# ziatdinovmax/GPim

Hardware: AMD Instinct MI355X
Metric: GP fit+predict grid-points/sec (higher is better)
Workload: dtype f64; 1 GPU; C2: 256x256 synthetic twisted-lattice image, 25% observed (N=16384, M=65536, d=2), Matern52 exact GP, T=100 Adam its (lr 0.1) + predict; one image per GPU; N=16384, M=65536, kernel=Matern52

## Files before the change

### gpim_amd/csrc/api.hip

```cpp
#include <math.h>
#include <stdio.h>
#include <string.h>
#include <stdlib.h>
#include <algorithm>
#include <chrono>
#include <atomic>
#include <mutex>
#include "common.hpp"
#include "border.hpp"
#include "vgp.hpp"
#include "sm.hpp"
#include "sample.hpp"
#include "acq.hpp"

static thread_local std::string g_err;
void gpim_set_error(const std::string& s) { g_err = s; }

int deal_chunk(int ntiles) { return std::max(1, std::min(64, ntiles / 512)); }
#define EAGER_MIN_PANELS 12


static inline int64_t mat_doubles(const gpimhip_ctx* h, int64_t elements) { return h->fp32 ? (elements + 1) / 2 : elements; }

static void ws_release_matrix(gpimhip_ctx* h) {
// ... 525 lines not shown
            if (graph) (void)hipGraphDestroy(graph);
            graph = nullptr;
            exec = nullptr;
            (void)hipGetLastError();
        }
    }
    RunAhead ra(h, h->np, loop.run_ahead);
    if (!exec) {
        for (int t = 0; t < T && !ra.stop(t); ++t) GP_TRY(iteration());
        return finish_and_check(h);
    }
    hipError_t le = hipSuccess;
    for (int t = 0; t < T && le == hipSuccess && !ra.stop(t); ++t) le = hipGraphLaunch(exec, h->stream);
    const int rc = finish_and_check(h);
    (void)hipGraphExecDestroy(exec);
    (void)hipGraphDestroy(graph);
    HIP_TRY(le);
    return rc;
}

extern "C" {

const char* gpimhip_last_error(void) { return g_err.c_str(); }

int gpimhip_shutdown(void) {
    std::lock_guard<std::mutex> lock(g_side_mutex);
    for (auto& S : g_side) {
        if (S.capture) (void)hipStreamDestroy(S.capture);
        S = SideStreams();
    }
    g_side_generation.fetch_add(1);
    return GPIMHIP_OK;
}
int gpimhip_version(void) { return 100; }

int gpimhip_create(gpimhip_handle* out, int device, void* hip_stream) {
    if (!out) return GPIMHIP_E_BADARG;
    HIP_TRY(hipSetDevice(device));
    gpimhip_ctx* h = new gpimhip_ctx();
    h->device = device;
    h->stream = (hipStream_t)hip_stream;
    int rc = GPIMHIP_OK;
    if ((rc = h->theta1.alloc(h, 1)) || (rc = h->info.alloc(h, 4))) {
        delete h;
        return rc;
    }
    (void)hipMemsetAsync(h->info, 0, 4 * sizeof(int32_t), h->stream);
    *out = h;
    return GPIMHIP_OK;
}

int gpimhip_set_precision(gpimhip_handle h, int32_t bits) {
    if (!h || (bits != 32 && bits != 64)) return GPIMHIP_E_BADARG;
    const int want = bits == 32 ? 1 : 0;
    if (want == h->fp32) return GPIMHIP_OK;
    if (want && h->refl.mask) {
        gpim_set_error("the symmetry-reduced model computes in double precision: leave reflection mode (gpimhip_set_reflection(h, 0, ...)) first");
        return GPIMHIP_E_BADARG;
    }
    HIP_TRY(hipSetDevice(h->device));
    HIP_TRY(hipStreamSynchronize(h->stream));
    ws_release_matrix(h);
    ws_release_predict(h);
    sample_release(h);
    ivr_release(h);
    h->fp32 = want;
    return GPIMHIP_OK;
}

int gpimhip_destroy(gpimhip_handle h) {
    if (!h) return GPIMHIP_OK;
    (void)hipSetDevice(h->device);
    (void)hipStreamSynchronize(h->stream);
    vfe_release(h);
    kron_release(h);
    vgp_release(h);
    pkron_release(h);
    sm_release(h);
    border_release(h);
    sample_release(h);
    ivr_release(h);
    ws_release_matrix(h);
    ws_release_predict(h);
    dev_release(h, h->keys, h->sel_scratch, h->acq_tmp, h->refine, h->bc, h->theta1, h->info, h->loo_tiles);
    if (h->plan.d_tiles) (void)hipFree(h->plan.d_tiles);
    step_plan_release(h);
    dist_plan_release(h);
    for (auto e : h->ra_ev)
        if (e) (void)hipEventDestroy(e);
    if (h->pinned_info) (void)hipHostFree(h->pinned_info);
    delete h;
    return GPIMHIP_OK;
}

int64_t gpimhip_workspace_bytes(gpimhip_handle h) {
    if (!h) return 0;
    const BorderWs* w = bws(h);
    return h->bytes + (w && w->sub ? w->sub->bytes : 0) + sample_bytes(h);
}

int gpimhip_timing_enable(gpimhip_handle h, int enable) {
    if (!h) return GPIMHIP_E_BADARG;
    h->timing = enable != 0;
    return GPIMHIP_OK;
}

int gpimhip_timing_read(gpimhip_handle h, int stage, double* total_ms, int64_t* count) {
    if (!h || stage < 0 || stage > 6 || !total_ms || !count) return GPIMHIP_E_BADARG;
    HIP_TRY(hipStreamSynchronize(h->stream));
    double tot = 0.0;
    for (auto& pr : h->ev[stage]) {
        float ms = 0.f;
        (void)hipEventElapsedTime(&ms, pr.first, pr.second);
        tot += ms;
        (void)hipEventDestroy(pr.first);
        (void)hipEventDestroy(pr.second);
    }
    *total_ms = tot;
    *count = (int64_t)h->ev[stage].size();
    h->ev[stage].clear();
    return GPIMHIP_OK;
}

int gpimhip_fit_completed(gpimhip_handle h) { return h ? h->fit_completed : 0; }

int gpimhip_sync(gpimhip_handle h) {
    if (!h) return GPIMHIP_E_BADARG;
    HIP_TRY(hipStreamSynchronize(h->stream));
    return GPIMHIP_OK;
}

int gpimhip_kmat(gpimhip_handle h, const gpimhip_model_t* m, const double* X, int64_t N, const double* Z,
                 int64_t M, const double* theta, double diag_add, double* out, int64_t ld) {
    FP64_ONLY(h);
    if (!h || !X || !theta || !out || N < 1) return GPIMHIP_E_BADARG;
    GP_TRY(check_model(m));
    HIP_TRY(hipSetDevice(h->device));
    const bool sym = (Z == nullptr);
    const int64_t Mv = sym ? N : M;
    if (Mv < 1 || ld < Mv) return GPIMHIP_E_BADARG;
    h->nbatch = 1;
    GP_TRY(launch_theta_raw(h, m, theta));
    const int64_t rp = pad_to(N, NB), cp = pad_to(Mv, NB);
    GP_TRY(ws_ensure_predict(h, rp, cp));
    const int64_t kld = h->ks_cols + 16;
    GP_TRY(launch_kmat(h, m, X, N, sym ? nullptr : Z, Mv, h->theta1, diag_add, 0, h->Ks, kld, rp, cp, sym ? 1 : 0, 0, 0,
                       0, 0));
    HIP_TRY(hipMemcpy2DAsync(out, (size_t)ld * sizeof(double), h->Ks, (size_t)kld * sizeof(double),
                             (size_t)Mv * sizeof(double), (size_t)N, hipMemcpyDeviceToDevice, h->stream));
    return GPIMHIP_OK;
}

int gpimhip_potrf(gpimhip_handle h, double* A, int64_t n, int64_t ld, int32_t* info) {
    FP64_ONLY(h);
    if (!h || !A || n < 1 || ld < n || !info) return GPIMHIP_E_BADARG;
    HIP_TRY(hipSetDevice(h->device));
    h->nbatch = 1;
    GP_TRY(ws_ensure(h, n));
    const int64_t np = h->np;
    HIP_TRY(hipMemsetAsync(info, 0, sizeof(int32_t), h->stream));
    GP_TRY(launch_pad_matrix_in(h, A, n, ld, h->A, np));
    GP_TRY(launch_potrf(h, h->A, np, np, info));
    GP_TRY(launch_pad_matrix_out_lower(h, h->A, np, A, n, ld));
    return GPIMHIP_OK;
}

static int fit_impl(gpimhip_ctx* h, const gpimhip_model_t* m, const double* X, int64_t x_bs, const double* y,
                    int64_t N, int B, double* u, double lr, int32_t T, double* hist_out, double* loss_out,
                    Objective obj = OBJ_NLL) {
    read_finalize_knob(h);
    HIP_TRY(hipSetDevice(h->device));
    h->nbatch = B;
    HIP_TRY(hipMemsetAsync(h->info, 0, sizeof(int32_t), h->stream));
    HIP_TRY(hipMemsetAsync(h->info + 1, 0x7f, sizeof(int32_t), h->stream));
    h->fit_completed = T;
    if (T == 0) return GPIMHIP_OK;
    GP_TRY(upload_bc_table(h, lr, T));
    if (use_small_path(N) && !h->refl.mask && obj == OBJ_NLL) {
        GP_TRY(launch_fit_small(h, m, X, x_bs, y, (int)N, u, h->bc, h->bc + T, T, hist_out, loss_out, nullptr));
        return finish_and_check(h);
    }
    GP_TRY(ws_ensure_padded(h, N));
    if (obj == OBJ_LOO) GP_TRY(loo_obj_ensure(h));
    if (border_on(h)) GP_TRY(border_ensure(h));
    HIP_TRY(hipMemsetAsync(h->adam_m, 0, (size_t)B * MAXP * sizeof(double), h->stream));
    HIP_TRY(hipMemsetAsync(h->adam_v, 0, (size_t)B * MAXP * sizeof(double), h->stream));
    HIP_TRY(hipMemsetAsync(h->iter, 0, (size_t)B * sizeof(int32_t), h->stream));
    HIP_TRY(hipMemsetAsync(h->fin_counter, 0, (size_t)B * sizeof(uint32_t), h->stream));
    GP_TRY(launch_pad_copy(h, y, N, h->ypad, h->np));
    const bool carry = !h->refl.mask && !h->no_fused_finalize;
    if (carry) GP_TRY(launch_theta(h, m, u));
    const IterTable tab{{h->iter, h->bc, T, hist_out, loss_out}, carry};
    const AdamStep st = adam_step_init();
    return run_fit_iterations(h, T, FIT_LOOP_DENSE,
                              [&] { return loss_grad_at_u(h, m, X, x_bs, N, u, 1, st, nullptr, nullptr, nullptr, &tab, obj); });
}


extern "C++" int64_t predict_chunk_cols(int64_t np, int B, int64_t M) {
    int64_t mc = std::min(pad_to(M, NB), std::max<int64_t>(NB, ((int64_t)1 << 27) / np / B / NB * NB));
    if (const char* e = getenv("GPIMHIP_PREDICT_CHUNK")) mc = std::min(mc, std::max<int64_t>(NB, atoll(e) / NB * NB));
    return mc;
}

extern "C++" int predict_cols(gpimhip_ctx* h, const PredictFamily& f, int64_t N, int B) {
    const int64_t np = h->np, M = f.M;
    const int nb = (int)(np / NB);
    if (f.fused && !h->fp32 && fused_predict_fits(np)) return f.fused();
    const int64_t mc = predict_chunk_cols(np, B, M);
    GP_TRY(ws_ensure_predict(h, np, mc));
    const bool bd = border_on(h);
    if (bd) GP_TRY(border_ensure_r(h, h->ks_cols));
    for (int64_t m0 = 0; m0 < M; m0 += mc) {
        const int64_t cnt = std::min(mc, M - m0), mcap = h->ks_cols;
        PredictChunk c{f.Xs + m0 * f.dim, m0, cnt, pad_to(cnt, NB), mcap, mcap + 16, cnt, nullptr};
        GP_TRY(f.slab(c));
        GP_TRY(launch_gemv_t(h, h->Ks, c.kld, np, c.cpad, h->alpha, h->mean_tmp, 0, np * c.kld, np, c.mcap));
        if (f.mean) GP_TRY(f.mean(c));
        if (f.var_on_domain && h->refl.var_count > 0 && !bd) c.nvar = std::max<int64_t>(0, std::min(cnt, h->refl.var_count - m0));
        if (c.nvar > 0) {
            GemmArgs g = gemm_args(h->A, h->ld, h->Ks, c.kld, nullptr, 0, 1.0, 0.0, h->pred_tiles, 0, h->np);
            if (c.nvar < c.cnt) g.cj_max = (int)((c.nvar + NB - 1) / NB);
            g.sB = np * c.kld;
            g.colpart = h->colpart;
            g.ld_colpart = c.mcap;
            g.sColpart = (int64_t)nb * c.mcap;
            g.ntiles = (int)h->pred_ntiles;
            g.chunk = deal_chunk(g.ntiles);
            g.rag = h->fp32 ? 0 : rag_of(N, np);
            { StageTimer t(h, 3); GP_TRY(launch_gemm(h, false, true, EPI_COLSUMSQ, g)); }
            if (bd) {
                BorderWs* w = bws(h);
                w->sub->stream = h->stream;
                const int64_t brows = (int64_t)(B / w->T) * np;
                GemmArgs gr = gemm_args(w->Y, w->mp, h->Ks, c.kld, w->R, w->r_cols, 1.0, 0.0, nullptr, 0, 0);
                gr.sA = brows * w->mp;
                gr.sB = brows * c.kld;
                gr.sC = w->mp * w->r_cols;
                gr.rect_rows = (int)(w->mp / NB);
                gr.rect_cols = (int)(c.cpad / NB);
                gr.ntiles = gr.rect_rows * gr.rect_cols;
                gr.kfix0 = 0;
                gr.kfix1 = (int)(brows / NB);
                gr.chunk = deal_chunk(gr.ntiles);
                GP_TRY(launch_gemm(w->sub, true, true, EPI_STORE, gr));
                GP_TRY(launch_border_colsumsq(h, w, c.cnt));
                c.radd = w->rsq;
            }
        }
        GP_TRY(f.finish(c));
    }
    return GPIMHIP_OK;
}

extern "C++" PredictFamily stationary_family(gpimhip_ctx* h, const gpimhip_model_t* m, const double* X, int64_t x_bs, int64_t N,
                                             int B, const double* Xs, int64_t M, double* mean_out, double* var_out) {
    PredictFamily f{m->dim, Xs, M};
    if (h->refl.mask) {
        const double scale = 1.0 / sqrt((double)(h->refl.nblocks_total > 0 ? h->refl.nblocks_total : B));
        f.var_on_domain = true;
        f.slab = [=](const PredictChunk& c) {
            return launch_kmat_refl(h, m, X, N, c.Z, c.cnt, h->theta, h->Ks, c.kld, h->np, c.cpad, 0, x_bs, 0, h->np * c.kld, scale);
        };
        f.finish = [=](const PredictChunk& c) {
            return launch_predict_coupled(h, c.mcap, (int)(h->np / NB), c.m0, c.cnt, c.nvar, c.mcap, mean_out, var_out, c.radd);
        };
        return f;
    }
    f.fused = [=] { return launch_predict_fused(h, m, X, x_bs, N, Xs, M, mean_out, var_out); };
    f.slab = [=](const PredictChunk& c) {
        return launch_kmat(h, m, X, N, c.Z, c.cnt, h->theta, 0.0, 0, h->Ks, c.kld, h->np, c.cpad, 0, 0, x_bs, 0, h->np * c.kld);
    };
    f.mean = [=](const PredictChunk& c) { return launch_copy_slice(h, h->mean_tmp, mean_out + c.m0, c.cnt, c.mcap, M); };
    f.finish = [=](const PredictChunk& c) { return launch_predict_var(h, c.mcap, (int)(h->np / NB), c.m0, c.cnt, var_out, M); };
    return f;
}

extern "C++" int model_state_at_u(gpimhip_ctx* h, const gpimhip_model_t* m, const double* X, int64_t x_bs, const double* y,
                                  int64_t N, int B, const double* u) {
    HIP_TRY(hipSetDevice(h->device));
    h->nbatch = B;
    GP_TRY(ws_ensure_padded(h, N));
    const int64_t np = h->np;
    HIP_TRY(hipMemsetAsync(h->info, 0, sizeof(int32_t), h->stream));
    GP_TRY(launch_pad_copy(h, y, N, h->ypad, np));
    if (border_on(h)) GP_TRY(border_ensure(h));
    GP_TRY(factor_at_u(h, m, X, x_bs, N, u));
    if (border_on(h)) {
        GP_TRY(launch_lauum(h, h->A, h->B, np, h->ld, rag_of(N, np)));
        GP_TRY(border_iter(h, N, false));
    }
    return GPIMHIP_OK;
}

static int predict_impl(gpimhip_ctx* h, const gpimhip_model_t* m, const double* X, int64_t x_bs, const double* y,
                        int64_t N, int B, const double* u, const double* Xs, int64_t M, double* mean_out,
                        double* var_out) {
    GP_TRY(model_state_at_u(h, m, X, x_bs, y, N, B, u));
    GP_TRY(predict_cols(h, stationary_family(h, m, X, x_bs, N, B, Xs, M, mean_out, var_out), N, B));
    return finish_and_check(h);
}

static int loss_grad_impl(gpimhip_ctx* h, const gpimhip_model_t* m, const double* X, const double* y, int64_t N, const double* u,
                          double* loss_out, double* grad_out, Objective obj) {
    read_finalize_knob(h);
    HIP_TRY(hipSetDevice(h->device));
    h->nbatch = 1;
    HIP_TRY(hipMemsetAsync(h->info, 0, sizeof(int32_t), h->stream));
    if (use_small_path(N) && obj == OBJ_NLL) {
        GP_TRY(launch_fit_small(h, m, X, 0, y, (int)N, const_cast<double*>(u), nullptr, nullptr, 0, nullptr,
                                loss_out, grad_out));
        return finish_and_check(h);
    }
    GP_TRY(ws_ensure_padded(h, N));
    if (obj == OBJ_LOO) GP_TRY(loo_obj_ensure(h));
    GP_TRY(launch_pad_copy(h, y, N, h->ypad, h->np));
    AdamStep st;
    memset(&st, 0, sizeof(st));
    GP_TRY(loss_grad_at_u(h, m, X, 0, N, const_cast<double*>(u), 0, st, loss_out, grad_out, nullptr, nullptr, obj));
    return finish_and_check(h);
}

int gpimhip_nll_grad(gpimhip_handle h, const gpimhip_model_t* m, const double* X, const double* y, int64_t N,
                     const double* u, double* loss_out, double* grad_out) {
    if (!h || !X || !y || !u || N < 1) return GPIMHIP_E_BADARG;
    GP_TRY(check_model(m));
    return loss_grad_impl(h, m, X, y, N, u, loss_out, grad_out, OBJ_NLL);
}

static int loo_objective_refused(const gpimhip_ctx* h, const char* who) {
    const char* why = h->fp32 ? "a single-precision handle (d = diag(S^-1) and the loss's log d cancel in float matrices: gpimhip_set_precision(h, 64))"
                    : border_on(h) ? "a border (the missing points couple the blocks: diag(S^-1) is no sum of the blocks' diagonals)"
                    : (h->refl.pb_off != 0 || h->refl.pb_stride != 1 || h->refl.raw || h->refl.nblocks_total) && h->refl.mask
                        ? "a shard of reflection blocks (the objective is not a sum over the blocks)"
                    : h->refl.mask ? "reflection mode (a lock-step batch of blocks: the held-out terms mix the blocks' diagonals)"
                                   : nullptr;
    if (!why) return GPIMHIP_OK;
    gpim_set_error(std::string(who) + ": the leave-one-out objective is the dense double-precision model's, one problem per call; refused on " + why);
    return GPIMHIP_E_BADARG;
}

int gpimhip_loo_grad(gpimhip_handle h, const gpimhip_model_t* m, const double* X, const double* y, int64_t N, const double* u,
                     double* loss_out, double* grad_out) {
    if (!h || !X || !y || !u || N < 1) return GPIMHIP_E_BADARG;
    GP_TRY(check_model(m));
    GP_TRY(loo_objective_refused(h, "gpimhip_loo_grad"));
    return loss_grad_impl(h, m, X, y, N, u, loss_out, grad_out, OBJ_LOO);
}

int gpimhip_fit_exact_loo(gpimhip_handle h, const gpimhip_model_t* m, const double* X, const double* y, int64_t N,
                          double* u_inout, double lr, int32_t T, double* hist_out, double* loss_out) {
    if (!h || !X || !y || !u_inout || N < 1 || T < 0) return GPIMHIP_E_BADARG;
    GP_TRY(check_model(m));
    GP_TRY(loo_objective_refused(h, "gpimhip_fit_exact_loo"));
    return fit_impl(h, m, X, 0, y, N, 1, u_inout, lr, T, hist_out, loss_out, OBJ_LOO);
}

int gpimhip_fit_exact(gpimhip_handle h, const gpimhip_model_t* m, const double* X, const double* y, int64_t N,
                      double* u_inout, double lr, int32_t T, double* hist_out, double* loss_out) {
    if (!h || !X || !y || !u_inout || N < 1 || T < 0) return GPIMHIP_E_BADARG;
    GP_TRY(check_model(m));
    return fit_impl(h, m, X, 0, y, N, 1, u_inout, lr, T, hist_out, loss_out);
}

int gpimhip_predict_exact(gpimhip_handle h, const gpimhip_model_t* m, const double* X, const double* y, int64_t N,
                          const double* u, const double* Xs, int64_t M, double* mean_out, double* var_out) {
    if (!h || !X || !y || !u || !Xs || M < 1 || N < 1 || !mean_out || !var_out) return GPIMHIP_E_BADARG;
    GP_TRY(check_model(m));
    return predict_impl(h, m, X, 0, y, N, 1, u, Xs, M, mean_out, var_out);
}

int gpimhip_fit_exact_batched(gpimhip_handle h, const gpimhip_model_t* m, const double* X, int64_t x_stride,
                              const double* y, int64_t N, int32_t B, double* u_inout, double lr, int32_t T,
                              double* hist_out, double* loss_out) {
    if (!h || !X || !y || !u_inout || N < 1 || T < 0 || B < 1 || B > 65535 ||
        (x_stride != 0 && x_stride < N * (m ? m->dim : 1)))
        return GPIMHIP_E_BADARG;
    GP_TRY(check_model(m));
    return fit_impl(h, m, X, x_stride, y, N, B, u_inout, lr, T, hist_out, loss_out);
}

int gpimhip_predict_exact_batched(gpimhip_handle h, const gpimhip_model_t* m, const double* X, int64_t x_stride,
// ... 137 lines not shown
```

### gpim_amd/csrc/common.hpp

```cpp
#pragma once
#include <hip/hip_runtime.h>
#include <stdint.h>
#include <functional>
#include <string>
#include <type_traits>
#include <vector>
#include <utility>
#include "../../include/gpimhip.h"

#define NB 128
#define GEMM_BK 16
#define MAXP GPIMHIP_MAX_PARAMS

void gpim_set_error(const std::string& s);

#define HIP_TRY(expr)                                                              \
    do {                                                                           \
        hipError_t _e = (expr);                                                    \
        if (_e != hipSuccess) {                                                    \
            gpim_set_error(std::string(#expr) + ": " + hipGetErrorString(_e));     \
            return GPIMHIP_E_HIP;                                                  \
        }                                                                          \
    } while (0)

// ... 97 lines not shown
    int64_t n_tiles = 0;
    std::vector<PlanRange> colfill;
    std::vector<PlanRange> upd_panel;
    std::vector<PlanRange> kinv_panel;
    PlanRange grad_tiles{0, 0};
    int rect_cols = 0;
    TileDesc* d_rect = nullptr;
    int64_t n_rect = 0;
};

struct ReflArgs {
    int mask;
    double twoc[GPIMHIP_MAX_DIM];
    const double* wts;
    int64_t n_total;
    int64_t var_count;
    int pb_off, pb_stride, nblocks_total, raw;
};
struct gpimhip_ctx {
    ReflArgs refl = {0, {0, 0, 0, 0}, nullptr, 0, 0, 0, 1, 0, 0};
    int device = 0;
    hipStream_t stream = nullptr;
    hipStream_t capture_stream = nullptr;
    bool capture_stream_tried = false;
    int side_generation = 0;
    int64_t np = 0;
    int64_t ld = 0;
    int nbatch = 1;
    int ws_batch = 0;
    DevBuf<double> A;
    DevBuf<double> B;
    DevBuf<double> Tm;
    DevBuf<double> dinv;
    DevBuf<double> dinvB;
    DevBuf<double> pcopy;
    DevBuf<double> ypad;
    DevBuf<double> z;
    DevBuf<double> alpha;
    DevBuf<double> logdet_part;
    DevBuf<double> grad_part;
    DevBuf<double> gemv_part;
    DevBuf<uint32_t> fin_counter;
    DevBuf<ThetaDev> theta;
    DevBuf<ThetaDev> theta1;
    DevBuf<int32_t> iter;
    DevBuf<double> adam_m;
    DevBuf<double> adam_v;
    DevBuf<int32_t> info;
    int64_t ks_rows = 0, ks_cols = 0, ks_batch = 0;
    struct PredList { int nc; DevBuf<TileDesc> tiles; };
    std::vector<PredList> pred_lists;
    DevBuf<double> Ks;
    DevBuf<double> colpart;
    DevBuf<double> mean_tmp;
    TileDesc* pred_tiles = nullptr;
    int64_t pred_ntiles = 0;
    int64_t bytes = 0;
    LinalgPlan plan;
    StepPlan splan, splan_inv;
    StepPlan splan_pair;
    DistPlan dplan;
    bool timing = false;
    std::vector<std::pair<hipEvent_t, hipEvent_t>> ev[7];
    DevBuf<double> bc;
    std::vector<double> bc_host;
    DevBuf<unsigned long long> keys;
    DevBuf<double> acq_tmp;
    DevBuf<char> sel_scratch;
    int fit_completed = 0;
    int32_t* pinned_info = nullptr;
    hipEvent_t ra_ev[2] = {nullptr, nullptr};
    void* vfe = nullptr;
    void* kron = nullptr;
    void* vgp = nullptr;
    void* pkron = nullptr;
    void* sm = nullptr;
    void* border = nullptr;
    void* sample = nullptr;
    void* ivr = nullptr;
    DevBuf<double> refine;
    DevBuf<double> loo_vec;
    DevBuf<TileDesc> loo_tiles;
    int loo_tiles_nb = 0;
    int fp32 = 0;
    bool no_fused_finalize = false;
};

template <typename T> int DevBuf<T>::alloc(gpimhip_ctx* h, int64_t count, const char* what) {
    void* q = nullptr;
    hipError_t e = hipMalloc(&q, (size_t)count * sizeof(T));
    if (e != hipSuccess) {
        if (what) (void)hipGetLastError();
        gpim_set_error(what ? std::string(what) : std::string("hipMalloc failed: ") + hipGetErrorString(e));
        return GPIMHIP_E_NOMEM;
    }
    p = (T*)q;
    cap = count;
    h->bytes += cap * (int64_t)sizeof(T);
    return GPIMHIP_OK;
}
template <typename T> void DevBuf<T>::release(gpimhip_ctx* h) {
    if (p) {
        (void)hipFree(p);
        h->bytes -= cap * (int64_t)sizeof(T);
    }
    p = nullptr;
    cap = 0;
}
template <typename T> int DevBuf<T>::grow(gpimhip_ctx* h, int64_t want) {
    if (cap >= want) return GPIMHIP_OK;
    HIP_TRY(hipStreamSynchronize(h->stream));
    release(h);
    return alloc(h, want);
}
template <typename... Bufs> static inline void dev_release(gpimhip_ctx* h, Bufs&... bufs) { (bufs.release(h), ...); }

struct BatchScope {
    gpimhip_ctx* h; int prev;
    BatchScope(gpimhip_ctx* h_, int nbatch) : h(h_), prev(h_->nbatch) { h->nbatch = nbatch; }
    ~BatchScope() { h->nbatch = prev; }
};

#define FP64_ONLY(h)                                                                                      \
    do {                                                                                                  \
        if ((h) && (h)->fp32) {                                                                           \
            gpim_set_error("this entry point needs a double-precision handle (gpimhip_set_precision(h, 64))"); \
            return GPIMHIP_E_BADARG;                                                                      \
        }                                                                                                 \
    } while (0)

static inline int64_t pad_to(int64_t n, int64_t m) { return (n + m - 1) / m * m; }
struct Carve {
    double* base;
    int64_t used = 0;
    explicit Carve(double* b) : base(b) {}
    template <typename T = double> T* take(int64_t doubles) {
        const int64_t off = (used + 1) & ~(int64_t)1;
        used = off + doubles;
        return base ? (T*)(base + off) : nullptr;
    }
};
static inline int rag_of(int64_t N, int64_t np) {
    const int64_t last = N - (np - NB);
    return (np >= 2 * NB && last > 0 && last <= 64) ? (int)(np / NB) : 0;
}

struct StageTimer {
    gpimhip_ctx* h; int stage; hipEvent_t e1 = nullptr;
    StageTimer(gpimhip_ctx* h_, int s) : h(h_), stage(s) {
        if (!h->timing) return;
        hipEvent_t e0;
        if (hipEventCreate(&e0) != hipSuccess || hipEventCreate(&e1) != hipSuccess) { e1 = nullptr; return; }
        (void)hipEventRecord(e0, h->stream);
        h->ev[stage].push_back({e0, e1});
    }
    ~StageTimer() { if (e1) (void)hipEventRecord(e1, h->stream); }
};

static inline int gemv_tri_rc(int64_t np) {
    const int64_t rc = ((np / 32 + NB - 1) / NB) * NB;
    return (int)(rc < NB ? NB : (rc > 1024 ? 1024 : rc));
}
static inline int gemv_tri_chunks(int64_t np) { return (int)((np + gemv_tri_rc(np) - 1) / gemv_tri_rc(np)); }
#define OUTER_W 4
int ws_ensure(gpimhip_ctx* h, int64_t N);
int ws_ensure_b(gpimhip_ctx* h, int64_t N, int B, int padded, bool matrices = true);
int ws_ensure_padded(gpimhip_ctx* h, int64_t N);
int ws_ensure_predict(gpimhip_ctx* h, int64_t np, int64_t mc);
int deal_chunk(int ntiles = 1 << 30);
void tri_tiles(std::vector<TileDesc>& tl, int nbr, int nc, bool lower);
void lower_patch_order(std::vector<TileDesc>& out, int lo, int hi, int kb0, int kb1);
int model_state_at_u(gpimhip_ctx* h, const gpimhip_model_t* m, const double* X, int64_t x_bs, const double* y, int64_t N,
                     int B, const double* u);
int solve_vectors(gpimhip_ctx* h, const gpimhip_model_t* m, const double* X, int64_t x_bs, int64_t N, bool defer_alpha = false);
int factor_at_u(gpimhip_ctx* h, const gpimhip_model_t* m, const double* X, int64_t x_bs, int64_t N, const double* u,
                bool theta_current = false, bool defer_alpha = false);
struct PredictChunk { const double* Z; int64_t m0, cnt, cpad, mcap, kld, nvar; const double* radd; };
struct PredictFamily {
    int dim; const double* Xs; int64_t M;
    bool var_on_domain = false;
    std::function<int()> fused;
    std::function<int(const PredictChunk&)> slab, mean, finish;
};
int64_t predict_chunk_cols(int64_t np, int B, int64_t M);
int predict_cols(gpimhip_ctx* h, const PredictFamily& f, int64_t N, int B);
PredictFamily stationary_family(gpimhip_ctx* h, const gpimhip_model_t* m, const double* X, int64_t x_bs, int64_t N, int B,
                                const double* Xs, int64_t M, double* mean_out, double* var_out);
void sample_release(gpimhip_ctx* h);
int64_t sample_bytes(const gpimhip_ctx* h);
void ivr_release(gpimhip_ctx* h);
int fit_prologue(gpimhip_ctx* h, double lr, int T, double* adam_m, double* adam_v, size_t adam_bytes, int32_t* iter);
int plan_ensure(gpimhip_ctx* h, int nb);
int check_model(const gpimhip_model_t* m);
int launch_potrf(gpimhip_ctx* h, double* A, int64_t np, int64_t ld, int32_t* info);
int launch_trtri(gpimhip_ctx* h, double* A, double* Tm, int64_t np, int64_t ld);
int launch_potrf_inv(gpimhip_ctx* h, double* A, double* Tm, int64_t np, int64_t ld, int32_t* info, int rag);
int launch_lauum(gpimhip_ctx* h, const double* A, double* B, int64_t np, int64_t ld, int rag);
int upload_bc_table(gpimhip_ctx* h, double lr, int T);
int finish_and_check(gpimhip_ctx* h);
struct FitLoop { bool dense_gates, run_ahead; };
static const FitLoop FIT_LOOP_DENSE = {true, true}, FIT_LOOP_PLAIN = {false, false};
int run_fit_iterations(gpimhip_ctx* h, int T, FitLoop loop, const std::function<int()>& iteration);
void vfe_release(gpimhip_ctx* h);
void kron_release(gpimhip_ctx* h);
void pkron_release(gpimhip_ctx* h);
int launch_potrf_steps(gpimhip_ctx* h, double* A, int64_t np, int64_t ld, int32_t* info, double* Tm = nullptr, int rag = 0);
int launch_potrf_steps_f32(gpimhip_ctx* h, double* A, int64_t np, int64_t ld, int32_t* info);
void step_plan_release(gpimhip_ctx* h);
int step_plan_ensure(gpimhip_ctx* h, int nb);
int step_plan_ensure_inv(gpimhip_ctx* h, int nb);
int step_plan_ensure_pair(gpimhip_ctx* h, int nb);
int launch_panel_chain(gpimhip_ctx* h, double* A, int64_t ld, int p0, int p1, int nb, const TileDesc* tiles,
                       const PlanRange* colfill, int32_t* info);
void dist_plan_release(gpimhip_ctx* h);
int launch_dist_pack(gpimhip_ctx* h, const double* P, int64_t ldp, int64_t r0, int64_t np, int w, const double* dinv,
                     int nblk, double* buf, int64_t ldb);
int launch_colsumsq_acc(gpimhip_ctx* h, const double* W, int64_t ldw, int rows, int64_t m, double* q);
int launch_dist_trsv(gpimhip_ctx* h, const double* P, int64_t ld, const double* D, int nblk, int backward, const double* r0,
                     const double* r1, double* out);
int launch_dist_rows_acc(gpimhip_ctx* h, const double* A, int64_t ld, int64_t rows, int w, const double* x, double* acc);
#define GEMV_T_MULTI_RC 1024
static inline int gemv_t_multi_chunks(int64_t nrows) { return (int)((nrows + GEMV_T_MULTI_RC - 1) / GEMV_T_MULTI_RC); }
int multi_group_width(int ncols);
int launch_dist_trsv_multi(gpimhip_ctx* h, const double* P, int64_t ld, const double* D, int nblk, int backward, const double* r0,
                           int64_t r0_cs, const double* r1, int64_t r1_cs, int64_t r1_chs, int nch, int ncols, double* out,
                           int64_t out_cs);
int launch_dist_rows_acc_multi(gpimhip_ctx* h, const double* A, int64_t ld, int64_t rows, int w, const double* x, int64_t x_cs,
                               int ncols, double* acc, int64_t acc_cs);
int launch_gemv_t_multi(gpimhip_ctx* h, const double* A, int64_t ld, int64_t nrows, int w, const double* x, int64_t x_cs,
                        int ncols, double* part);
int launch_theta_raw(gpimhip_ctx* h, const gpimhip_model_t* m, const double* raw);
int launch_kmat(gpimhip_ctx* h, const gpimhip_model_t* m, const double* X, int64_t N, const double* Z,
                int64_t M, const ThetaDev* theta, double diag_add, int use_theta_diag, double* out,
                int64_t ld, int64_t rows_pad, int64_t cols_pad, int sym, int lower_only, int64_t x_bs,
                int64_t z_bs, int64_t out_bs);
int launch_pad_copy(gpimhip_ctx* h, const double* src, int64_t n, double* dst, int64_t np);
int launch_diag_inv_copy(gpimhip_ctx* h, double* A, int64_t ld, int nb);
int launch_pad_matrix_in(gpimhip_ctx* h, const double* src, int64_t n, int64_t ld, double* dst, int64_t np);
int launch_pad_matrix_out_lower(gpimhip_ctx* h, const double* src, int64_t np, double* dst, int64_t n, int64_t ld);
int launch_trmv_lower(gpimhip_ctx* h, const double* L, int64_t ld, int64_t np, const double* y, double* z);
int launch_gemv_t(gpimhip_ctx* h, const double* A, int64_t ld, int64_t nrows, int64_t ncols, const double* x,
                  double* out, int tri, int64_t a_bs, int64_t x_bs, int64_t o_bs);
int launch_kres(gpimhip_ctx* h, const gpimhip_model_t* m, const double* X, int64_t x_bs, int64_t N, double* scratch,
                int S, double* res);
int launch_axpy(gpimhip_ctx* h, double* x, const double* d, int64_t n);
int launch_gemv_t_tri(gpimhip_ctx* h, const double* A, int64_t ld, int64_t np, const double* x, double* part, double* out);
int launch_kmat_refl(gpimhip_ctx* h, const gpimhip_model_t* m, const double* X, int64_t N, const double* Z, int64_t M,
                     const ThetaDev* theta, double* out, int64_t ld, int64_t rows_pad, int64_t cols_pad, int sym, int64_t x_bs,
                     int64_t z_bs, int64_t out_bs, double scale);
int launch_add_diag_theta(gpimhip_ctx* h, double* out, int64_t ld, int64_t row0, int64_t n, int64_t npad);
int launch_theta(gpimhip_ctx* h, const gpimhip_model_t* m, const double* u);
int launch_grad_reduce(gpimhip_ctx* h, const gpimhip_model_t* m, const double* Kinv, int64_t ld,
                       const double* X, int64_t N, int nb, const double* alpha, int64_t x_bs);
int launch_grad_reduce_fin(gpimhip_ctx* h, const gpimhip_model_t* m, const double* X, int64_t x_bs, int64_t N,
                           bool alpha_deferred, double* u, int do_adam, AdamStep st, const FinalizeOut& out, int carry_theta);
int launch_finalize(gpimhip_ctx* h, const gpimhip_model_t* m, int64_t N, int64_t np, double* u, int do_adam,
                    AdamStep st, const FinalizeOut& out, int carry_theta = 0);
int launch_finalize_vec(gpimhip_ctx* h, const gpimhip_model_t* m, int64_t N, int64_t np, double* u, int do_adam, AdamStep st,
                        const FinalizeOut& out, int carry_theta, const double* z, const double* zb);
int launch_grad_reduce_loo(gpimhip_ctx* h, const gpimhip_model_t* m, const double* Kinv, int64_t ld, const double* X, int64_t N,
                           int nb, const double* alpha, const double* rvec);
int loo_obj_ensure(gpimhip_ctx* h);
int loo_grad_at_u(gpimhip_ctx* h, const gpimhip_model_t* m, const double* X, int64_t N, double* u, int do_adam, AdamStep st,
                  const FinalizeOut& out, bool theta_carried);
int launch_grad_reduce_tiles(gpimhip_ctx* h, const gpimhip_model_t* m, const double* Kinv, int64_t ld, const double* X,
                             int64_t N, int64_t np, const double* alpha, const TileDesc* tiles, int ntile, double* part);
int launch_sum7(gpimhip_ctx* h, const double* part, int ntile, double* S);
int launch_grad_reduce_refl(gpimhip_ctx* h, const gpimhip_model_t* m, const double* Kinv, int64_t ld, const double* X,
                            int64_t N, int nb, const double* alpha, int64_t x_bs);
int launch_finalize_coupled(gpimhip_ctx* h, const gpimhip_model_t* m, int64_t N, int64_t np, double* u, int do_adam,
                            AdamStep st, const FinalizeOut& out, const double* border_scal = nullptr);
int launch_coupled_sums(gpimhip_ctx* h, int64_t np, double* out11);
int launch_dist_finalize_dev(gpimhip_ctx* h, const gpimhip_model_t* m, int64_t N, const double* red, const double* quad,
                             double* u, int do_adam, AdamStep st, double* loss_out, double* grad_out, double* hist_row);
int launch_dist_finalize(gpimhip_ctx* h, const gpimhip_model_t* m, int64_t N, const double* S, double q2, double lg,
                         double* u, int do_adam, AdamStep st, double* loss_out, double* grad_out, double* hist_row);
int launch_predict_var(gpimhip_ctx* h, int64_t ldp, int nb, int64_t m0, int64_t mcount, double* var_out, int64_t M);
int launch_copy_slice(gpimhip_ctx* h, const double* src, double* dst, int64_t n, int64_t s_bs, int64_t d_bs);
int launch_predict_coupled(gpimhip_ctx* h, int64_t ldp, int nb, int64_t m0, int64_t mcount, int64_t nvar, int64_t mean_bs,
                           double* mean_out, double* var_out, const double* radd = nullptr);
struct LooSrc {
    const double* y; const double* diag_part; int nR, rc; int64_t np; const double* alpha;
    int B; const double* wts; const int32_t* rep; const int32_t* sgn; int64_t Nq;
};
static inline int loo_blocks(int64_t n) { return n > 1024 * 256 ? 1024 : (int)((n + 255) / 256); }
int launch_colsq_tri(gpimhip_ctx* h, const double* A, int64_t ld, int64_t np, int64_t N, double* part);
int launch_loo_finish(gpimhip_ctx* h, const LooSrc& s, int64_t n, const ThetaDev* theta, double* part, double* mean_out,
                      double* var_out, double* score_out);
int launch_acq(gpimhip_ctx* h, int kind, const double* mean, const double* sd, int64_t M, double p0, double p1,
               const double* mask, double* out);
int launch_nanmax(gpimhip_ctx* h, const double* x, int64_t n, double* out);
int launch_topk(gpimhip_ctx* h, const double* x, int64_t M, int k, int keep_nan, double* vals, int64_t* idx,
                int64_t* count);
int launch_topk_radix(gpimhip_ctx* h, const double* x, int64_t M, int k, int keep_nan, double* vals, int64_t* idx,
                      int64_t* count);
int launch_nanmax_two_stage(gpimhip_ctx* h, const double* x, int64_t n, double* out);
int launch_thin_batch(gpimhip_ctx* h, const double* vals, const int64_t* flat, int n, int d, const int64_t* shape,
                      double dscale, int max_out, int32_t* keep_out, int32_t* nkeep_out);
size_t sel_scratch_bytes();
int sel_scratch_ensure(gpimhip_ctx* h);
int launch_fit_small(gpimhip_ctx* h, const gpimhip_model_t* m, const double* X, int64_t x_bs, const double* y,
                     int N, double* u, const double* lr_over_bc1, const double* bc2_sqrt, int T, double* hist,
                     double* loss, double* grad);
bool fused_predict_fits(int64_t np);


enum GemmEpi { EPI_STORE = 0, EPI_COLSUMSQ = 1 };
struct GemmArgs {
    const double* A; int64_t lda; int a_roff, a_coff;
    const double* B; int64_t ldb; int b_roff, b_coff;
    double* C; int64_t ldc; int c_roff, c_coff;
    double alpha, beta;
    const TileDesc* tiles; int ntiles;
    int cj_max;
    int cmap;
    int chunk;
    int inplace;
    int rag;
    int krev;
    int kfix0, kfix1;
    int rect_rows, rect_cols;
    double* colpart; int64_t ld_colpart;
    double* C2;
    int shape_div;
    int64_t sA, sB, sC, sColpart;
    int bshift;
};
int launch_gemm(gpimhip_ctx* h, bool a_km, bool b_km, int epi, const GemmArgs& g);
int launch_gemm_f32(gpimhip_ctx* h, bool a_km, bool b_km, int epi, const GemmArgs& g);
GemmArgs gemm_args(const double* A, int64_t lda, const double* B, int64_t ldb, double* C, int64_t ldc, double alpha, double beta,
                   const TileDesc* tiles, int n, int64_t rows);

enum GemmShape {
    GEMM_SHAPE_QUAD = GPIMHIP_GEMM_SHAPE_QUAD,
    GEMM_SHAPE_ROWHALF = GPIMHIP_GEMM_SHAPE_ROWHALF,
    GEMM_SHAPE_8W_LDS = GPIMHIP_GEMM_SHAPE_8W_LDS,
    GEMM_SHAPE_8W = GPIMHIP_GEMM_SHAPE_8W,
    GEMM_SHAPE_4W = GPIMHIP_GEMM_SHAPE_4W
};
static inline bool gemm_layout_ok(bool a_km, bool b_km, int epi) {
    if (epi == EPI_STORE) return !a_km || b_km;
    return epi == EPI_COLSUMSQ && !a_km && b_km;
}
int gemm_shape_f64(bool a_km, bool b_km, int epi, int64_t ntiles, int64_t batch, int shape_div, int inplace);
int gemm_shape_f32(bool a_km, bool b_km, int epi, int64_t ntiles, int64_t batch, int shape_div, int inplace);
int gemm_tile_pos_f32(int n, int chunk, int quads, int bx, int& quad);

template <int TSM, int TSN>
__host__ __device__ __forceinline__ int gemm_tile_pos(int n, int chunk, int bx, int& quad) {
    constexpr int QUADS = (128 / TSM) * (128 / TSN);
    const int b = bx / QUADS;
    quad = bx % QUADS;
    if (QUADS > 1) return b;
    if (chunk == 0) {
        const int q = n >> 3, r = n & 7, x = b & 7, yy = b >> 3;
        return (x < r ? x * (q + 1) : r * (q + 1) + (x - r) * q) + yy;
    }
    const int C = chunk, full = (n / (8 * C)) * (8 * C);
    if (b < full) {
        const int x = b & 7, y = b >> 3, round = y / C;
        return (round * 8 + ((round & 1) ? 7 - x : x)) * C + (y % C);
    }
    return b;
}
__host__ __device__ __forceinline__ void gemm_rect_tile(int rect_rows, int rect_cols, int p, int& ci, int& cj) {
    const int per = 8 * rect_cols, s = p / per, q = p - s * per, left = rect_rows - 8 * s, rows_here = left < 8 ? left : 8;
    ci = 8 * s + q % rows_here;
    cj = q / rows_here;
}
```

### gpim_amd/csrc/predict.hip

```cpp
#include "kfun.hpp"
#include "tile128.hpp"
#include "acq.hpp"

typedef double d4 __attribute__((ext_vector_type(4)));

#define PF_CT 32
#define PF_LDK (PF_CT + 16)

struct FusedPredictArgs {
    const double* X; int64_t N; int64_t x_bs; int d;
    const double* Xs; int64_t M;
    const ThetaDev* th;
    const double* Linv; int64_t ld; int64_t np;
    const double* alpha;
    double* mean_out; double* var_out;
    AcqOut acq;
};

template <int KIND>
__global__ __launch_bounds__(256, 2) void predict_fused_kernel(FusedPredictArgs a) {
    extern __shared__ __attribute__((aligned(16))) double smem[];
    const int np = (int)a.np;
    double* Ks = smem;
    double* xa = smem + (size_t)np * PF_LDK;
// ... 240 lines not shown
    if (rp == 0) red[wave][cp] = v;
    __syncthreads();
    if (threadIdx.x < 32) {
        d2 t = red[0][cp];
        t[0] = ((t[0] + red[1][cp][0]) + red[2][cp][0]) + red[3][cp][0];
        t[1] = ((t[1] + red[1][cp][1]) + red[2][cp][1]) + red[3][cp][1];
        *reinterpret_cast<d2*>(part + (int64_t)cb * 64 + 2 * cp) = t;
    }
}
int launch_colsq_tri(gpimhip_ctx* h, const double* A, int64_t ld, int64_t np, int64_t N, double* part) {
    const int rc = gemv_tri_rc(np), nR = gemv_tri_chunks(np);
    const dim3 grid((unsigned)((np / 64) * nR), h->nbatch);
    if (h->fp32)
        hipLaunchKernelGGL(colsq_tri_kernel<float>, grid, dim3(256), 0, h->stream, reinterpret_cast<const float*>(A), ld, np, N,
                           part, rc, nR, np * ld);
    else
        hipLaunchKernelGGL(colsq_tri_kernel<double>, grid, dim3(256), 0, h->stream, A, ld, np, N, part, rc, nR, np * ld);
    HIP_TRY(hipGetLastError());
    return GPIMHIP_OK;
}

__global__ __launch_bounds__(256) void loo_finish_kernel(LooSrc s, int64_t n, const ThetaDev* __restrict__ th,
                                                         double* __restrict__ mean_out, double* __restrict__ var_out,
                                                         double* __restrict__ part) {
    __shared__ double red[256];
    const double noise = th->noise, dadd = th->diag_add;
    double elpd = 0.0, sse = 0.0;
    for (int64_t i = (int64_t)blockIdx.x * 256 + threadIdx.x; i < n; i += (int64_t)gridDim.x * 256) {
        double d = 0.0, a = 0.0;
        if (s.B == 0) {
            d = gemv_tri_alpha(s.diag_part, s.nR, s.rc, s.np, i);
            a = s.alpha[i];
        } else {
            const int64_t p = s.rep[i];
            const int g = s.sgn[i];
            const double sb = sqrt((double)s.B);
            for (int b = 0; b < s.B; ++b) {
                const double w = s.wts ? s.wts[(int64_t)b * s.Nq + p] : 1.0;
                if (w == 0.0) continue;
                const double c = 1.0 / (w * sb);
                d = fma(c * c, gemv_tri_alpha(s.diag_part + (int64_t)b * s.nR * s.np, s.nR, s.rc, s.np, p), d);
                const double t = c * s.alpha[(int64_t)b * s.np + p];
                a += (__popc(b & g) & 1) ? -t : t;
            }
        }
        const double yi = s.y[i];
        const double mu = yi - a / d, v = clamp0_nan(1.0 / d - dadd) + noise;
        const double res = yi - mu;
        mean_out[i] = mu;
        var_out[i] = v;
        elpd -= 0.5 * (log(6.283185307179586476925 * v) + res * res / v);
        sse = fma(res, res, sse);
    }
    elpd = block_sum_256(elpd, red);
    sse = block_sum_256(sse, red);
    if (threadIdx.x == 0) {
        part[2 * blockIdx.x] = elpd;
        part[2 * blockIdx.x + 1] = sse;
    }
}
__global__ __launch_bounds__(256) void loo_score_kernel(const double* __restrict__ part, int nblk, double* __restrict__ score) {
    __shared__ double red[256];
    double elpd = 0.0, sse = 0.0;
    for (int k = threadIdx.x; k < nblk; k += 256) {
        elpd += part[2 * k];
        sse += part[2 * k + 1];
    }
    elpd = block_sum_256(elpd, red);
    sse = block_sum_256(sse, red);
    if (threadIdx.x == 0) {
        score[0] = elpd;
        score[1] = sse;
    }
}
int launch_loo_finish(gpimhip_ctx* h, const LooSrc& s, int64_t n, const ThetaDev* theta, double* part, double* mean_out,
                      double* var_out, double* score_out) {
    const int nblk = loo_blocks(n);
    hipLaunchKernelGGL(loo_finish_kernel, dim3(nblk), dim3(256), 0, h->stream, s, n, theta, mean_out, var_out, part);
    HIP_TRY(hipGetLastError());
    hipLaunchKernelGGL(loo_score_kernel, dim3(1), dim3(256), 0, h->stream, (const double*)part, nblk, score_out);
    HIP_TRY(hipGetLastError());
    return GPIMHIP_OK;
}
```

Before: 8921 grid-points/s.

## Skip variance GEMM for prediction points coincident with training inputs

Before prediction, a matching kernel finds which test points exactly equal a training input. Those points are compacted to the end of the prediction set, and the expensive variance GEMM runs only on the unmatched points. Variance at coincident points is then filled in from a triangular column-sum via a closed-form expression. This cuts variance work when the prediction grid contains the training points, as in this benchmark where 25% are observed. The cost is an O(N*M) matching pass, a host sync, and scatter and compaction kernels.

Result: no change. 8999 grid-points/s, median of 6 (+0.9%).

```diff
diff --git a/gpim_amd/csrc/api.hip b/gpim_amd/csrc/api.hip
--- a/gpim_amd/csrc/api.hip
+++ b/gpim_amd/csrc/api.hip
@@ -631,7 +631,7 @@
     ivr_release(h);
     ws_release_matrix(h);
     ws_release_predict(h);
-    dev_release(h, h->keys, h->sel_scratch, h->acq_tmp, h->refine, h->bc, h->theta1, h->info, h->loo_tiles);
+    dev_release(h, h->keys, h->sel_scratch, h->acq_tmp, h->refine, h->bc, h->theta1, h->info, h->loo_tiles, h->coin_idx, h->coin_scr);
     if (h->plan.d_tiles) (void)hipFree(h->plan.d_tiles);
     step_plan_release(h);
     dist_plan_release(h);
@@ -756,7 +756,7 @@
     const int64_t np = h->np, M = f.M;
     const int nb = (int)(np / NB);
     if (f.fused && !h->fp32 && fused_predict_fits(np)) return f.fused();
-    const int64_t mc = predict_chunk_cols(np, B, M);
+    const int64_t mc = predict_chunk_cols(np, B, f.chunk_for > 0 ? f.chunk_for : M);
     GP_TRY(ws_ensure_predict(h, np, mc));
     const bool bd = border_on(h);
     if (bd) GP_TRY(border_ensure_r(h, h->ks_cols));
@@ -767,9 +767,10 @@
         GP_TRY(launch_gemv_t(h, h->Ks, c.kld, np, c.cpad, h->alpha, h->mean_tmp, 0, np * c.kld, np, c.mcap));
         if (f.mean) GP_TRY(f.mean(c));
         if (f.var_on_domain && h->refl.var_count > 0 && !bd) c.nvar = std::max<int64_t>(0, std::min(cnt, h->refl.var_count - m0));
+        if (f.var_count >= 0) c.nvar = std::max<int64_t>(0, std::min(cnt, f.var_count - m0));
         if (c.nvar > 0) {
             GemmArgs g = gemm_args(h->A, h->ld, h->Ks, c.kld, nullptr, 0, 1.0, 0.0, h->pred_tiles, 0, h->np);
-            if (c.nvar < c.cnt) g.cj_max = (int)((c.nvar + NB - 1) / NB);
+            if (c.nvar < c.cnt || f.chunk_for > 0) g.cj_max = (int)((c.nvar + NB - 1) / NB);
             g.sB = np * c.kld;
             g.colpart = h->colpart;
             g.ld_colpart = c.mcap;
@@ -821,7 +822,9 @@
         return launch_kmat(h, m, X, N, c.Z, c.cnt, h->theta, 0.0, 0, h->Ks, c.kld, h->np, c.cpad, 0, 0, x_bs, 0, h->np * c.kld);
     };
     f.mean = [=](const PredictChunk& c) { return launch_copy_slice(h, h->mean_tmp, mean_out + c.m0, c.cnt, c.mcap, M); };
-    f.finish = [=](const PredictChunk& c) { return launch_predict_var(h, c.mcap, (int)(h->np / NB), c.m0, c.cnt, var_out, M); };
+    f.finish = [=](const PredictChunk& c) {
+        return c.nvar > 0 ? launch_predict_var(h, c.mcap, (int)(h->np / NB), c.m0, c.nvar, var_out, M) : GPIMHIP_OK;
+    };
     return f;
 }
 
@@ -842,11 +845,57 @@
     return GPIMHIP_OK;
 }
 
+static void read_coincident_knob(gpimhip_ctx* h) { h->no_coincident = getenv("GPIMHIP_NO_COINCIDENT") != nullptr; }
+static int64_t coincident_min_np() {
+    const char* e = getenv("GPIMHIP_COINCIDENT_MIN_NP");
+    return e ? atoll(e) : 16 * NB;
+}
+
 static int predict_impl(gpimhip_ctx* h, const gpimhip_model_t* m, const double* X, int64_t x_bs, const double* y,
                         int64_t N, int B, const double* u, const double* Xs, int64_t M, double* mean_out,
                         double* var_out) {
+    read_coincident_knob(h);
+    const int64_t E = M / NB * NB;
+    bool coin = !h->no_coincident && B == 1 && !h->fp32 && !h->refl.mask && E > 0 && M < ((int64_t)1 << 31) - 256 && N < ((int64_t)1 << 31);
+    if (coin) {
+        HIP_TRY(hipSetDevice(h->device));
+        h->nbatch = B;
+        GP_TRY(ws_ensure_padded(h, N));
+        coin = !fused_predict_fits(h->np) && h->np >= coincident_min_np();
+    }
+    int64_t Mu = E;
+    CoinIdx ci;
+    double *Xc = nullptr, *mean_c = nullptr, *var_c = nullptr;
+    if (coin) {
+        GP_TRY(h->coin_idx.grow(h, CoinIdx::size(M)));
+        GP_TRY(h->coin_scr.grow(h, M * (m->dim + 2)));
+        ci = CoinIdx(h->coin_idx, M);
+        Xc = h->coin_scr;
+        mean_c = Xc + M * m->dim;
+        var_c = mean_c + M;
+        GP_TRY(launch_coincident_match(h, X, N, Xs, M, m->dim, ci, Xc));
+        int32_t counts[2] = {0, 0};
+        HIP_TRY(hipMemcpyAsync(counts, ci.counts, sizeof(counts), hipMemcpyDeviceToHost, h->stream));
+        HIP_TRY(hipStreamSynchronize(h->stream));
+        Mu = counts[0];
+    }
     GP_TRY(model_state_at_u(h, m, X, x_bs, y, N, B, u));
-    GP_TRY(predict_cols(h, stationary_family(h, m, X, x_bs, N, B, Xs, M, mean_out, var_out), N, B));
+    if (Mu == E) {
+        GP_TRY(predict_cols(h, stationary_family(h, m, X, x_bs, N, B, Xs, M, mean_out, var_out), N, B));
+        return finish_and_check(h);
+    }
+    PredictFamily f = stationary_family(h, m, X, x_bs, N, B, Xc, E, mean_c, var_c);
+    f.var_count = Mu;
+    f.chunk_for = M;
+    GP_TRY(predict_cols(h, f, N, B));
+    if (M > E) {
+        PredictFamily t = stationary_family(h, m, X, x_bs, N, B, Xc + E * m->dim, M - E, mean_c + E, var_c + E);
+        t.chunk_for = M;
+        GP_TRY(predict_cols(h, t, N, B));
+    }
+    GP_TRY(launch_coincident_scatter(h, ci, M, Mu, mean_c, var_c, mean_out, var_out));
+    GP_TRY(launch_colsq_tri(h, h->A, h->ld, h->np, N, h->gemv_part));
+    GP_TRY(launch_coincident_closed(h, m, ci, M, h->gemv_part, var_out));
     return finish_and_check(h);
 }
 
diff --git a/gpim_amd/csrc/common.hpp b/gpim_amd/csrc/common.hpp
--- a/gpim_amd/csrc/common.hpp
+++ b/gpim_amd/csrc/common.hpp
@@ -203,6 +203,9 @@
     DevBuf<double> loo_vec;
     DevBuf<TileDesc> loo_tiles;
     int loo_tiles_nb = 0;
+    DevBuf<int32_t> coin_idx;
+    DevBuf<double> coin_scr;
+    bool no_coincident = false;
     int fp32 = 0;
     bool no_fused_finalize = false;
 };
@@ -300,6 +303,8 @@
 struct PredictFamily {
     int dim; const double* Xs; int64_t M;
     bool var_on_domain = false;
+    int64_t var_count = -1;
+    int64_t chunk_for = 0;
     std::function<int()> fused;
     std::function<int(const PredictChunk&)> slab, mean, finish;
 };
@@ -408,6 +413,20 @@
 int launch_colsq_tri(gpimhip_ctx* h, const double* A, int64_t ld, int64_t np, int64_t N, double* part);
 int launch_loo_finish(gpimhip_ctx* h, const LooSrc& s, int64_t n, const ThetaDev* theta, double* part, double* mean_out,
                       double* var_out, double* score_out);
+struct CoinIdx {
+    int32_t *match = nullptr, *umap = nullptr, *blk = nullptr, *counts = nullptr; int nblk = 0;
+    CoinIdx() {}
+    CoinIdx(int32_t* base, int64_t M) : match(base), umap(base + M), blk(base + 2 * M), nblk((int)((M + 255) / 256)) {
+        counts = blk + 2 * (int64_t)nblk;
+    }
+    static int64_t size(int64_t M) { return 2 * M + 2 * ((M + 255) / 256) + 2; }
+};
+int launch_coincident_match(gpimhip_ctx* h, const double* X, int64_t N, const double* Xs, int64_t M, int d, const CoinIdx& ci,
+                            double* Xc);
+int launch_coincident_scatter(gpimhip_ctx* h, const CoinIdx& ci, int64_t M, int64_t Mu, const double* mean_c, const double* var_c,
+                              double* mean_out, double* var_out);
+int launch_coincident_closed(gpimhip_ctx* h, const gpimhip_model_t* m, const CoinIdx& ci, int64_t M, const double* part,
+                             double* var_out);
 int launch_acq(gpimhip_ctx* h, int kind, const double* mean, const double* sd, int64_t M, double p0, double p1,
                const double* mask, double* out);
 int launch_nanmax(gpimhip_ctx* h, const double* x, int64_t n, double* out);
diff --git a/gpim_amd/csrc/predict.hip b/gpim_amd/csrc/predict.hip
--- a/gpim_amd/csrc/predict.hip
+++ b/gpim_amd/csrc/predict.hip
@@ -346,3 +346,142 @@
     HIP_TRY(hipGetLastError());
     return GPIMHIP_OK;
 }
+
+#define COIN_TILE 1024
+#define COIN_ROWS 4096
+template <int D>
+__global__ __launch_bounds__(256) void coincident_match_kernel(const double* __restrict__ X, int64_t N, const double* __restrict__ Xs,
+                                                               int64_t M, int32_t* __restrict__ match) {
+    __shared__ double xt[COIN_TILE * D];
+    const int64_t j = (int64_t)blockIdx.x * 256 + threadIdx.x;
+    double t[D];
+#pragma unroll
+    for (int k = 0; k < D; ++k) t[k] = j < M ? Xs[j * D + k] : __longlong_as_double(0x7ff8000000000000ll);
+    const int64_t r0 = (int64_t)blockIdx.y * COIN_ROWS, r1 = r0 + COIN_ROWS < N ? r0 + COIN_ROWS : N;
+    int64_t best = -1;
+    for (int64_t b0 = r0; b0 < r1; b0 += COIN_TILE) {
+        const int cnt = (int)(r1 - b0 < COIN_TILE ? r1 - b0 : COIN_TILE);
+        __syncthreads();
+        for (int e = threadIdx.x; e < cnt * D; e += 256) xt[e] = X[b0 * D + e];
+        __syncthreads();
+        int hit = -1;
+#pragma unroll 8
+        for (int i = cnt - 1; i >= 0; --i) {
+            bool eq = xt[i * D] == t[0];
+#pragma unroll
+            for (int k = 1; k < D; ++k) eq = eq && (xt[i * D + k] == t[k]);
+            hit = eq ? i : hit;
+        }
+        if (best < 0 && hit >= 0) best = b0 + hit;
+    }
+    if (j < M && best >= 0) atomicMin(reinterpret_cast<unsigned int*>(match) + j, (unsigned int)best);
+}
+__global__ __launch_bounds__(256) void coincident_count_kernel(const int32_t* __restrict__ match, int64_t E, int32_t* __restrict__ blk) {
+    const int64_t j = (int64_t)blockIdx.x * 256 + threadIdx.x;
+    const int c = __syncthreads_count(j < E && match[j] < 0);
+    if (threadIdx.x == 0) blk[blockIdx.x] = c;
+}
+__global__ __launch_bounds__(256) void coincident_scan_kernel(const int32_t* __restrict__ blk, int nblk, int32_t* __restrict__ off,
+                                                              int32_t* __restrict__ counts, int64_t E) {
+    __shared__ int sh[256];
+    int carry = 0;
+    for (int b0 = 0; b0 < nblk; b0 += 256) {
+        const int b = b0 + threadIdx.x;
+        const int v = b < nblk ? blk[b] : 0;
+        sh[threadIdx.x] = v;
+        __syncthreads();
+        for (int s = 1; s < 256; s <<= 1) {
+            const int t = (int)threadIdx.x >= s ? sh[threadIdx.x - s] : 0;
+            __syncthreads();
+            sh[threadIdx.x] += t;
+            __syncthreads();
+        }
+        if (b < nblk) off[b] = carry + sh[threadIdx.x] - v;
+        carry += sh[255];
+        __syncthreads();
+    }
+    if (threadIdx.x == 0) {
+        counts[0] = carry;
+        counts[1] = (int32_t)(E - carry);
+    }
+}
+__global__ __launch_bounds__(256) void coincident_gather_kernel(const int32_t* __restrict__ match, int64_t M, int64_t E,
+                                                                const int32_t* __restrict__ off, const int32_t* __restrict__ counts,
+                                                                const double* __restrict__ Xs, int d, int32_t* __restrict__ umap,
+                                                                double* __restrict__ Xc) {
+    __shared__ int wsum[4];
+    const int64_t j = (int64_t)blockIdx.x * 256 + threadIdx.x;
+    const bool un = j < E && match[j] < 0;
+    const unsigned long long bal = __ballot(un);
+    const int lane = threadIdx.x & 63, wave = threadIdx.x >> 6;
+    if (lane == 0) wsum[wave] = __popcll(bal);
+    __syncthreads();
+    int64_t nun = off[blockIdx.x] + __popcll(bal & ((1ull << lane) - 1ull));
+    for (int w = 0; w < wave; ++w) nun += wsum[w];
+    if (j < M) {
+        const int64_t p = j >= E ? j : (un ? nun : counts[0] + (j - nun));
+        umap[p] = (int32_t)j;
+        for (int k = 0; k < d; ++k) Xc[p * d + k] = Xs[j * d + k];
+    }
+}
+__global__ __launch_bounds__(256) void coincident_scatter_kernel(const int32_t* __restrict__ umap, int64_t M, int64_t E, int64_t Mu,
+                                                                 const double* __restrict__ mean_c, const double* __restrict__ var_c,
+                                                                 double* __restrict__ mean_out, double* __restrict__ var_out) {
+    const int64_t p = (int64_t)blockIdx.x * 256 + threadIdx.x;
+    if (p >= M) return;
+    const int64_t j = umap[p];
+    mean_out[j] = mean_c[p];
+    if (p < Mu || p >= E) var_out[j] = var_c[p];
+}
+template <int KIND>
+__global__ __launch_bounds__(256) void coincident_closed_kernel(const int32_t* __restrict__ match, int64_t E,
+                                                                const double* __restrict__ part, int nR, int rc, int64_t np,
+                                                                const ThetaDev* __restrict__ th, double* __restrict__ var_out) {
+    const int64_t j = (int64_t)blockIdx.x * 256 + threadIdx.x;
+    if (j >= E) return;
+    const int64_t i = match[j];
+    if (i < 0) return;
+    const double s = th->diag_add, d = gemv_tri_alpha(part, nR, rc, np, i);
+    const double k0 = th->var * kfun_value<KIND>(0.0, th->alpha);
+    var_out[j] = clamp0_nan((th->var - k0) + fma(-(s * s), d, s)) + th->noise;
+}
+
+int launch_coincident_match(gpimhip_ctx* h, const double* X, int64_t N, const double* Xs, int64_t M, int d, const CoinIdx& ci,
+                            double* Xc) {
+    HIP_TRY(hipMemsetAsync(ci.match, 0xff, (size_t)M * sizeof(int32_t), h->stream));
+    const dim3 grid((unsigned)ci.nblk, (unsigned)((N + COIN_ROWS - 1) / COIN_ROWS));
+    switch (d) {
+    case 1: hipLaunchKernelGGL(coincident_match_kernel<1>, grid, dim3(256), 0, h->stream, X, N, Xs, M, ci.match); break;
+    case 2: hipLaunchKernelGGL(coincident_match_kernel<2>, grid, dim3(256), 0, h->stream, X, N, Xs, M, ci.match); break;
+    case 3: hipLaunchKernelGGL(coincident_match_kernel<3>, grid, dim3(256), 0, h->stream, X, N, Xs, M, ci.match); break;
+    case 4: hipLaunchKernelGGL(coincident_match_kernel<4>, grid, dim3(256), 0, h->stream, X, N, Xs, M, ci.match); break;
+    default: return GPIMHIP_E_BADARG;
+    }
+    HIP_TRY(hipGetLastError());
+    const int64_t E = M / NB * NB;
+    hipLaunchKernelGGL(coincident_count_kernel, dim3(ci.nblk), dim3(256), 0, h->stream, ci.match, E, ci.blk);
+    HIP_TRY(hipGetLastError());
+    hipLaunchKernelGGL(coincident_scan_kernel, dim3(1), dim3(256), 0, h->stream, ci.blk, ci.nblk, ci.blk + ci.nblk, ci.counts, E);
+    HIP_TRY(hipGetLastError());
+    hipLaunchKernelGGL(coincident_gather_kernel, dim3(ci.nblk), dim3(256), 0, h->stream, ci.match, M, E, ci.blk + ci.nblk, ci.counts, Xs,
+                       d, ci.umap, Xc);
+    HIP_TRY(hipGetLastError());
+    return GPIMHIP_OK;
+}
+int launch_coincident_scatter(gpimhip_ctx* h, const CoinIdx& ci, int64_t M, int64_t Mu, const double* mean_c, const double* var_c,
+                              double* mean_out, double* var_out) {
+    hipLaunchKernelGGL(coincident_scatter_kernel, dim3((unsigned)ci.nblk), dim3(256), 0, h->stream, ci.umap, M, M / NB * NB, Mu, mean_c,
+                       var_c, mean_out, var_out);
+    HIP_TRY(hipGetLastError());
+    return GPIMHIP_OK;
+}
+int launch_coincident_closed(gpimhip_ctx* h, const gpimhip_model_t* m, const CoinIdx& ci, int64_t M, const double* part,
+                             double* var_out) {
+    return with_kind(m->kernel, [&](auto K) {
+        constexpr int KIND = decltype(K)::value;
+        hipLaunchKernelGGL(coincident_closed_kernel<KIND>, dim3((unsigned)ci.nblk), dim3(256), 0, h->stream, ci.match, M / NB * NB,
+                           part, gemv_tri_chunks(h->np), gemv_tri_rc(h->np), h->np, h->theta, var_out);
+        HIP_TRY(hipGetLastError());
+        return GPIMHIP_OK;
+    });
+}
```
